# bentherien/point-cloud-reid

Hardware: AMD Instinct MI355X
Metric: siamese pair-comparisons/sec @1024 pts (higher is better)
Workload: dtype bf16x3

## Files before the change

point-cloud-reid_amd/csrc/attn_kernels_impl.h:

```cpp
#pragma once
#ifndef PCR_ATTN_PREC
#define PCR_ATTN_PREC 0
#endif
#include "tile_dense.h"

#include <stdio.h>

#include <vector>

namespace {
constexpr int kAPrec = PCR_ATTN_PREC;
struct AttnArgs {
  pcr_attn_params p;
  int dbg;
};

constexpr int kATraceWgs = 512, kATraceRecs = 24, kATraceMarks = 8;
__device__ unsigned long long g_attn_trace[2 * kATraceWgs * kATraceRecs * kATraceMarks];


__device__ __forceinline__ void pos_hidden(float *dst, int RP, const float *P, const float *w0,
                                           const float *b0, int d, int T) {
  for (int e = threadIdx.x; e < d * T; e += blockDim.x) {
    const int o = e / T, t = e - o * T;
// ... 1051 lines not shown
      bf_split8(xv, bh[s2], bl[s2], true);
    }
    PCR_AMARK(1);
    f32x16 q[ND];
#pragma unroll
    for (int cb = 0; cb < ND; cb++)
#pragma unroll
      for (int r = 0; r < 16; r++) q[cb][r] = 0.f;
    {
      const bf16x8 *wb = s_wq + lane;
#pragma unroll
      for (int s2 = 0; s2 < SQ; s2++) {
        bf16x8 wh[ND], wl[ND];
#pragma unroll
        for (int cb = 0; cb < ND; cb++) {
          wh[cb] = wb[((s2 * ND + cb) * 2) * 64];
          wl[cb] = wb[((s2 * ND + cb) * 2 + 1) * 64];
        }
#pragma unroll
        for (int cb = 0; cb < ND; cb++) q[cb] = __builtin_amdgcn_mfma_f32_32x32x16_bf16(wh[cb], bh[s2], q[cb], 0, 0, 0);
#pragma unroll
        for (int cb = 0; cb < ND; cb++) q[cb] = __builtin_amdgcn_mfma_f32_32x32x16_bf16(wh[cb], bl[s2], q[cb], 0, 0, 0);
#pragma unroll
        for (int cb = 0; cb < ND; cb++) q[cb] = __builtin_amdgcn_mfma_f32_32x32x16_bf16(wl[cb], bh[s2], q[cb], 0, 0, 0);
      }
    }
    PCR_AMARK(2);
    bf16x8 mh[SD][ND], ml[SD][ND];
    {
      const bf16x8 *mb = reinterpret_cast<const bf16x8 *>(kvp) + lane;
#pragma unroll
      for (int s2 = 0; s2 < SD; s2++)
#pragma unroll
        for (int cb = 0; cb < ND; cb++) {
          mh[s2][cb] = mb[((s2 * ND + cb) * 2) * 64];
          ml[s2][cb] = mb[((s2 * ND + cb) * 2 + 1) * 64];
        }
    }
    __builtin_amdgcn_fence(__ATOMIC_RELEASE, "wavefront");
    __builtin_amdgcn_wave_barrier();
    __builtin_amdgcn_fence(__ATOMIC_ACQUIRE, "wavefront");
    float z16[2][2] = {{0.f, 0.f}, {0.f, 0.f}};
#pragma unroll
    for (int cb = 0; cb < ND; cb++)
#pragma unroll
      for (int g = 0; g < 4; g++) {
        const f32x4 bqv = cvec(s_c, cb, g), ksv = cvec(ksw, cb, g);
        float zz = 0.f;
#pragma unroll
        for (int qq = 0; qq < 4; qq++) {
          const float v = elu1(q[cb][4 * g + qq] + bqv[qq]);
          q[cb][4 * g + qq] = v;
          zz += v * ksv[qq];
        }
        if ((g & 1) == 0) z16[cb][g >> 1] = zz;
        else z16[cb][g >> 1] += zz;
      }
    float zs[2][2];
    {
      float za = z16[0][0], zb = z16[0][1], zc = z16[1][0], zd = z16[1][1];
      if (dh >= 32) {
        za += zb; zb = za;
        zc += zd; zd = zc;
      }
      if (ND == 2 && dh >= 64) {
        za += zc; zb = za; zc = za; zd = za;
      }
      za += __shfl_xor(za, 32, 64);
      zb += __shfl_xor(zb, 32, 64);
      zc += __shfl_xor(zc, 32, 64);
      zd += __shfl_xor(zd, 32, 64);
      zs[0][0] = (1.0f / (za + 1e-6f)) * skf;
      zs[0][1] = (1.0f / (zb + 1e-6f)) * skf;
      zs[1][0] = (1.0f / (zc + 1e-6f)) * skf;
      zs[1][1] = (1.0f / (zd + 1e-6f)) * skf;
    }
#pragma unroll
    for (int cb = 0; cb < ND; cb++)
#pragma unroll
      for (int r = 0; r < 16; r++) q[cb][r] *= zs[cb][r >> 3];
    bf16x8 ch_[SD], cl_[SD];
#pragma unroll
    for (int cb = 0; cb < ND; cb++)
#pragma unroll
      for (int G = 0; G < 2; G++) to_ops(q[cb], G, ch_[2 * cb + G], cl_[2 * cb + G]);
    f32x16 m[ND];
#pragma unroll
    for (int cb = 0; cb < ND; cb++)
#pragma unroll
      for (int r = 0; r < 16; r++) m[cb][r] = 0.f;
#pragma unroll
    for (int s2 = 0; s2 < SD; s2++) {
#pragma unroll
      for (int cb = 0; cb < ND; cb++) m[cb] = __builtin_amdgcn_mfma_f32_32x32x16_bf16(mh[s2][cb], ch_[s2], m[cb], 0, 0, 0);
#pragma unroll
      for (int cb = 0; cb < ND; cb++) m[cb] = __builtin_amdgcn_mfma_f32_32x32x16_bf16(mh[s2][cb], cl_[s2], m[cb], 0, 0, 0);
#pragma unroll
      for (int cb = 0; cb < ND; cb++) m[cb] = __builtin_amdgcn_mfma_f32_32x32x16_bf16(ml[s2][cb], ch_[s2], m[cb], 0, 0, 0);
    }
    auto layernorm = [&](auto &v, auto nb_tag, const float *gam, const float *bet) __attribute__((always_inline)) {
      constexpr int NB = decltype(nb_tag)::value;
      float sm = 0.f;
#pragma unroll
      for (int cb = 0; cb < NB; cb++)
#pragma unroll
        for (int r = 0; r < 16; r++) sm += v[cb][r];
      sm += __shfl_xor(sm, 32, 64);
      const float mean = sm / (32.0f * NB);
      float vr = 0.f;
#pragma unroll
      for (int cb = 0; cb < NB; cb++)
#pragma unroll
        for (int r = 0; r < 16; r++) {
          const float dlt = v[cb][r] - mean;
          vr += dlt * dlt;
        }
      vr += __shfl_xor(vr, 32, 64);
      const float inv = 1.0f / sqrtf(vr / (32.0f * NB) + 1e-5f);
#pragma unroll
      for (int cb = 0; cb < NB; cb++)
#pragma unroll
        for (int g = 0; g < 4; g++) {
          const f32x4 gv = cvec(gam, cb, g), bv = cvec(bet, cb, g);
#pragma unroll
          for (int qq = 0; qq < 4; qq++) v[cb][4 * g + qq] = (v[cb][4 * g + qq] - mean) * inv * gv[qq] + bv[qq];
        }
    };
    PCR_AMARK(3);
    layernorm(m, std::integral_constant<int, ND>{}, s_c + 64, s_c + 128);
    PCR_AMARK(4);
#pragma unroll
    for (int s2 = 0; s2 < C1S; s2++) {
      float xv[8];
#pragma unroll
      for (int e = 0; e < 8; e++) xv[e] = xf[8 * s2 + e];
      bf_split8(xv, bh[s2], bl[s2], true);
    }
#pragma unroll
    for (int cb = 0; cb < ND; cb++)
#pragma unroll
      for (int G = 0; G < 2; G++) to_ops(m[cb], G, bh[C1S + 2 * cb + G], bl[C1S + 2 * cb + G]);
    f32x16 f[SD];
#pragma unroll
    for (int cb = 0; cb < SD; cb++)
#pragma unroll
      for (int r = 0; r < 16; r++) f[cb][r] = 0.f;
    {
      const bf16x8 *wb = s_w0 + lane;
#pragma unroll
      for (int s2 = 0; s2 < S0; s2++) {
        bf16x8 wh[SD], wl[SD];
#pragma unroll
        for (int cb = 0; cb < SD; cb++) {
          wh[cb] = wb[((s2 * SD + cb) * 2) * 64];
          wl[cb] = wb[((s2 * SD + cb) * 2 + 1) * 64];
        }
#pragma unroll
        for (int cb = 0; cb < SD; cb++) f[cb] = __builtin_amdgcn_mfma_f32_32x32x16_bf16(wh[cb], bh[s2], f[cb], 0, 0, 0);
#pragma unroll
        for (int cb = 0; cb < SD; cb++) f[cb] = __builtin_amdgcn_mfma_f32_32x32x16_bf16(wh[cb], bl[s2], f[cb], 0, 0, 0);
#pragma unroll
        for (int cb = 0; cb < SD; cb++) f[cb] = __builtin_amdgcn_mfma_f32_32x32x16_bf16(wl[cb], bh[s2], f[cb], 0, 0, 0);
      }
    }
#pragma unroll
    for (int cb = 0; cb < SD; cb++) {
#pragma unroll
      for (int r = 0; r < 16; r++) f[cb][r] = relu_i(f[cb][r]);
#pragma unroll
      for (int G = 0; G < 2; G++) to_ops(f[cb], G, bh[2 * cb + G], bl[2 * cb + G]);
    }
    PCR_AMARK(5);
    f32x16 o[NOB];
#pragma unroll
    for (int cb = 0; cb < NOB; cb++)
#pragma unroll
      for (int r = 0; r < 16; r++) o[cb][r] = 0.f;
    {
      const bf16x8 *wb = s_w2 + lane;
#pragma unroll
      for (int s2 = 0; s2 < 4 * ND; s2++) {
        bf16x8 wh[NOB], wl[NOB];
#pragma unroll
        for (int cb = 0; cb < NOB; cb++) {
          wh[cb] = wb[((s2 * NOB + cb) * 2) * 64];
          wl[cb] = wb[((s2 * NOB + cb) * 2 + 1) * 64];
        }
#pragma unroll
        for (int cb = 0; cb < NOB; cb++) o[cb] = __builtin_amdgcn_mfma_f32_32x32x16_bf16(wh[cb], bh[s2], o[cb], 0, 0, 0);
#pragma unroll
        for (int cb = 0; cb < NOB; cb++) o[cb] = __builtin_amdgcn_mfma_f32_32x32x16_bf16(wh[cb], bl[s2], o[cb], 0, 0, 0);
#pragma unroll
        for (int cb = 0; cb < NOB; cb++) o[cb] = __builtin_amdgcn_mfma_f32_32x32x16_bf16(wl[cb], bh[s2], o[cb], 0, 0, 0);
      }
    }
    PCR_AMARK(6);
    layernorm(o, std::integral_constant<int, NOB>{}, s_c + 192, s_c + 192 + 32 * NOB);
    if constexpr (C1S == 2 * NOB) {
      if (p.residual) {
#pragma unroll
        for (int cb = 0; cb < NOB; cb++)
#pragma unroll
          for (int r = 0; r < 16; r++) o[cb][r] += xf[16 * cb + r];
      }
    }
    if constexpr (POOL) {
      float vm[16], vs[16];
      {
        const bool up = (j & 1) != 0;
#pragma unroll
        for (int r = 0; r < 16; r++) {
          const float lo_ = o[r >> 4][r & 15], hi_ = o[(r + 16) >> 4][(r + 16) & 15];
          const float tk = up ? hi_ : lo_, uk = up ? lo_ : hi_;
          const float pu = __uint_as_float(pcr_sort_partner<2, 1>(__float_as_uint(uk), lane));
          vm[r] = fmaxf(tk, pu);
          vs[r] = tk + pu;
        }
      }
#define PCR_POOL_STEP(N, J, BIT)                                                                      \
      {                                                                                               \
        const bool up = (j & BIT) != 0;                                                               \
        _Pragma("unroll") for (int r = 0; r < N; r++) {                                               \
          const float tm = up ? vm[r + N] : vm[r], um = up ? vm[r] : vm[r + N];                       \
          const float ts = up ? vs[r + N] : vs[r], us = up ? vs[r] : vs[r + N];                       \
          vm[r] = fmaxf(tm, __uint_as_float(pcr_sort_partner<2 * J, J>(__float_as_uint(um), lane)));  \
          vs[r] = ts + __uint_as_float(pcr_sort_partner<2 * J, J>(__float_as_uint(us), lane));        \
        }                                                                                             \
      }
      PCR_POOL_STEP(8, 2, 2)
      PCR_POOL_STEP(4, 4, 4)
      PCR_POOL_STEP(2, 8, 8)
      PCR_POOL_STEP(1, 16, 16)
#undef PCR_POOL_STEP
      pmax = fmaxf(pmax, vm[0]);
      psum += vs[0];
      if (++pblk == nblk) {
        const int e = ((j & 1) << 4) | ((j & 2) << 2) | (j & 4) | ((j & 8) >> 2) | ((j & 16) >> 4);
        const int ch = 16 * (e >> 3) + bf_kpos(h, e & 7);
        float *po = p.pool_out + (size_t)b * 128;
        po[ch] = pmax;
        po[64 + ch] = psum;
        pmax = -INFINITY;
        psum = 0.f;
        pblk = 0;
        pc += nwav;
      }
    } else if constexpr (!CF) {
      const __amdgpu_buffer_rsrc_t rout =
          __builtin_amdgcn_make_buffer_rsrc(p.out + (size_t)b * (32 * NOB) * p.Lq, 0, 32 * NOB * p.Lq * 4, 0x00020000);
#pragma unroll
      for (int e = 0; e < 16 * NOB; e++) {
        const int ch = 16 * (e >> 3) + bf_kpos(0, e & 7);
        const float v = o[e >> 4][e & 15];
        __builtin_amdgcn_raw_buffer_store_b32(__builtin_bit_cast(unsigned, v), rout, vo, ch * p.Lq * 4, 0);
      }
    } else {
#pragma unroll
      for (int cb = 0; cb < NOB; cb++)
#pragma unroll
        for (int G = 0; G < 2; G++) to_ops(o[cb], G, bh[2 * cb + G], bl[2 * cb + G]);
      f32x16 fo[CF ? CF : 1];
#pragma unroll
      for (int cb = 0; cb < CF; cb++)
#pragma unroll
        for (int r = 0; r < 16; r++) fo[cb][r] = 0.f;
      const bf16x8 *wb = reinterpret_cast<const bf16x8 *>(p.wfinal) + lane;
#pragma unroll
      for (int s2 = 0; s2 < 2 * NOB; s2++) {
        bf16x8 wh[CF ? CF : 1], wl[CF ? CF : 1];
#pragma unroll
        for (int cb = 0; cb < CF; cb++) {
          wh[cb] = wb[((s2 * CF + cb) * 2) * 64];
          wl[cb] = wb[((s2 * CF + cb) * 2 + 1) * 64];
        }
#pragma unroll
        for (int cb = 0; cb < CF; cb++) fo[cb] = __builtin_amdgcn_mfma_f32_32x32x16_bf16(wh[cb], bh[s2], fo[cb], 0, 0, 0);
#pragma unroll
        for (int cb = 0; cb < CF; cb++) fo[cb] = __builtin_amdgcn_mfma_f32_32x32x16_bf16(wh[cb], bl[s2], fo[cb], 0, 0, 0);
#pragma unroll
        for (int cb = 0; cb < CF; cb++) fo[cb] = __builtin_amdgcn_mfma_f32_32x32x16_bf16(wl[cb], bh[s2], fo[cb], 0, 0, 0);
      }
      const __amdgpu_buffer_rsrc_t rout =
          __builtin_amdgcn_make_buffer_rsrc(p.out + (size_t)b * (32 * CF) * p.Lq, 0, 32 * CF * p.Lq * 4, 0x00020000);
#pragma unroll
      for (int cb = 0; cb < CF; cb++)
#pragma unroll
        for (int g = 0; g < 4; g++) {
          const f32x4 bv = cvec(s_c + 320, cb, g);
#pragma unroll
          for (int qq = 0; qq < 4; qq++) {
            const int e = 16 * cb + 4 * g + qq;
            const int ch = 16 * (e >> 3) + bf_kpos(0, e & 7);
            const float v = fo[cb][4 * g + qq] + bv[qq];
            __builtin_amdgcn_raw_buffer_store_b32(__builtin_bit_cast(unsigned, v), rout, vo, ch * p.Lq * 4, 0);
          }
        }
    }
    __builtin_amdgcn_wave_barrier();
    PCR_AMARK(7);
    PCR_ANEXT();
  }
#undef PCR_AMARK
#undef PCR_ANEXT
}
#endif

}

static int attn_check(const pcr_attn_params &p) {
  if (p.B < 0 || p.Lq < 1 || p.Sk < 1 || p.c1 < 1 || p.c2 < 1 || p.cout < 1 || p.nhead < 1) return 1;
  if (p.d < 32 || p.d > 512 || (p.d & 31) || p.d % p.nhead) return 1;
  if (p.d > 128 && ((p.d & 63) || ((p.d / p.nhead) & 63) || p.d / p.nhead > 256)) return 1;
  if ((p.c2 & 7) || p.cout > 512 || p.cfinal > 512) return 1;
  if (!p.feat_q || !p.feat_k || !p.xyz_k || !p.kv || !p.pos0_w || !p.pos0_b || !p.wq || !p.bq || !p.wkv ||
      !p.bkv || !p.wmerge || !p.wmlp0 || !p.wmlp2 || !p.ln1_g || !p.ln1_b || !p.ln2_g || !p.ln2_b)
    return 1;
  if (p.q_pos && (!p.xyz_q || p.c1 != p.c2 || p.c1 != p.d)) return 1;
  if (p.residual && p.cout != p.c1) return 1;
  if (p.cfinal && (!p.wfinal || !p.bfinal || (p.cout & 7))) return 1;
  return 0;
}

static void attn_dump_trace(const char *path, const char *tag, int wgs, int B, int Sk) {
  static int launches = 0;
  static const int skip = pcr_tune_int("PCR_SA_TRACE_SKIP");
  launches++;
  if (launches <= skip || launches > skip + 8) return;
  static std::vector<unsigned long long> host(2 * kATraceWgs * kATraceRecs * kATraceMarks);
  if (hipDeviceSynchronize() != hipSuccess) return;
  if (hipMemcpyFromSymbol(host.data(), HIP_SYMBOL(g_attn_trace), host.size() * sizeof(unsigned long long)) != hipSuccess) return;
  FILE *f = fopen(path, "a");
  if (!f) return;
  const int n = 2 * (wgs < kATraceWgs ? wgs : kATraceWgs);
  fprintf(f, "launch %d kernel %s wgs %d B %d Sk %d\n", launches, tag, wgs, B, Sk);
  for (int w = 0; w < n; w++) {
    const unsigned long long *t = host.data() + (size_t)w * (kATraceRecs * kATraceMarks);
    fprintf(f, "wg %d", w);
    for (int i = 0; i < kATraceRecs * kATraceMarks; i++) fprintf(f, " %llu", t[i]);
    fprintf(f, "\n");
  }
  fclose(f);
}

static int attn_kv_narrow(const pcr_attn_params *pp, pcr_stream_t stream) {
  AttnArgs a;
  a.p = *pp;
  a.dbg = 0;
  const int d = pp->d;
  if (pp->c2 < pp->d) return PCR_ERR_INVALID;
  const int tb = d <= 64 ? 2 : 1, RP = 32 * tb + 1;
  size_t lds = (size_t)(pp->c2 + d + 3) * RP + 4 * d;
  const size_t lds2 = (size_t)d * (d + 1) + d;
  if (lds2 > lds) lds = lds2;
  lds = (lds + kThreads) * sizeof(float);
  if (lds > (size_t)kMaxDynLds) return PCR_ERR_INVALID;
  static bool ok = allow_big_lds(attn_kv_kernel<2, 1, 2, 1>) && allow_big_lds(attn_kv_kernel_o3<2, 1, 1, 1>) &&
                   allow_big_lds(attn_kv_kernel_o3<1, 2, 1, 4>) && allow_big_lds(attn_kv_kernel<1, 2, 0, 4>);
  (void)ok;
  const int ntile = (pp->Sk + 32 * tb - 1) / (32 * tb);
  int ns = pp->kv_splits > 1 ? pp->kv_splits : 1;
  if (ns > 1 && (!pp->kv_part || ns > 64)) return PCR_ERR_INVALID;
  if (ns > ntile) ns = ntile;
  a.p.kv_splits = ns;
  dim3 g(pp->B, ns), blk(kThreads);
  hipStream_t st = pcr_s(stream);
  constexpr bool kBfUnit = kAPrec != 0;
  const bool bfk = kBfUnit && pp->wkv_bf != nullptr;
  if (ns == 1 && d == 64 && (pp->c2 == 64 || (pp->c2 == 128 && bfk && pp->Sk >= 128)) && (pp->Sk & 31) == 0 && pp->nhead >= 1 &&
      64 % pp->nhead == 0) {
    const bool bf = bfk;
    const bool wide = pp->c2 == 128;
    pcr_note_arith(bf ? PCR_PREC_BF16X3 : PCR_PREC_F32);
    static bool oks = allow_big_lds(attn_kv_stream64_kernel<true, false>) && allow_big_lds(attn_kv_stream64_kernel<false, false>) &&
                      allow_big_lds(attn_kv_stream64_kernel<true, kBfUnit>) && allow_big_lds(attn_kv_stream64_kernel<false, kBfUnit>) &&
                      allow_big_lds(attn_kv_stream64_kernel<true, kBfUnit, kBfUnit ? 8 : 4>) &&
                      allow_big_lds(attn_kv_stream64_kernel<false, kBfUnit, kBfUnit ? 8 : 4>);
    (void)oks;
    const int nblk = pp->Sk >> 5;
    const int minw = wide ? 4 : 2;
    int wpc2 = 1;
    while (wpc2 * 2 <= (nblk < 4 ? nblk : 4)) wpc2 *= 2;
    if (wpc2 < minw) wpc2 = minw;
    static const int no_onew = pcr_tune_int("PCR_ATTN_NO_ONEW");
    const bool onew = kBfUnit && bf && !wide && nblk <= 4 && !no_onew;
    if (onew) wpc2 = 1;
    const int cpg = kKvsWaves / wpc2;
    const size_t wu = bf ? (size_t)((wide ? 8 : 4) + 4) * 512 : 4096;
    const size_t lds_s = (wu * 4 + 256 + 128 + 64 * 65 + (onew ? (size_t)0 : (size_t)cpg * (64 * 65 + 64))) * sizeof(float);
    const long rounds = ((long)pp->B + cpg - 1) / cpg;
    static const int ncu = [] {
      hipDeviceProp_t pr;
      int dev = 0;
      if (hipGetDevice(&dev) != hipSuccess || hipGetDeviceProperties(&pr, dev) != hipSuccess) return 256;
      return pr.multiProcessorCount > 0 ? pr.multiProcessorCount : 256;
    }();
    const int gs = (int)(rounds < ncu ? rounds : ncu);
    const dim3 gg(gs), bb(64 * kKvsWaves);
    if (bf && wide) {
      if (pp->nhead >= 2) hipLaunchKernelGGL((attn_kv_stream64_kernel<true, kBfUnit, kBfUnit ? 8 : 4>), gg, bb, lds_s, st, a);
      else hipLaunchKernelGGL((attn_kv_stream64_kernel<false, kBfUnit, kBfUnit ? 8 : 4>), gg, bb, lds_s, st, a);
    } else if (bf) {
      static const char *atrace = pcr_tune_str("PCR_ATTN_TRACE");
      if (atrace) a.dbg |= 256;
      if (onew) {
        static bool oko = allow_big_lds(attn_kv_stream64_kernel<true, kBfUnit, 4, kBfUnit>) &&
                          allow_big_lds(attn_kv_stream64_kernel<false, kBfUnit, 4, kBfUnit>);
        (void)oko;
        if (pp->nhead >= 2) hipLaunchKernelGGL((attn_kv_stream64_kernel<true, kBfUnit, 4, kBfUnit>), gg, bb, lds_s, st, a);
        else hipLaunchKernelGGL((attn_kv_stream64_kernel<false, kBfUnit, 4, kBfUnit>), gg, bb, lds_s, st, a);
      } else if (pp->nhead >= 2) hipLaunchKernelGGL((attn_kv_stream64_kernel<true, kBfUnit>), gg, bb, lds_s, st, a);
      else hipLaunchKernelGGL((attn_kv_stream64_kernel<false, kBfUnit>), gg, bb, lds_s, st, a);
      if (atrace) attn_dump_trace(atrace, "kv64", gs, (int)pp->B, pp->Sk);
    } else {
      if (pp->nhead >= 2) hipLaunchKernelGGL((attn_kv_stream64_kernel<true, false>), gg, bb, lds_s, st, a);
      else hipLaunchKernelGGL((attn_kv_stream64_kernel<false, false>), gg, bb, lds_s, st, a);
    }
    PCR_CHECK_LAUNCH();
    return PCR_OK;
  }
#if PCR_ATTN_PREC != 0
  if (ns == 1 && d == 32 && pp->c2 == 32 && pp->wkv_bf && (pp->Sk & 31) == 0 && pp->nhead >= 1 && 32 % pp->nhead == 0) {
    static bool ok32 = allow_big_lds(attn_kv_stream32_kernel);
    (void)ok32;
    pcr_note_arith(PCR_PREC_BF16X3);
    const int nblk = pp->Sk >> 5;
    int wpc2 = 1;
    while (wpc2 * 2 <= (nblk < kKvsWaves ? nblk : kKvsWaves)) wpc2 *= 2;
    if (wpc2 < 2) wpc2 = 2;
    const int cpg = kKvsWaves / wpc2;
    const size_t lds_s = (size_t)(4096 + 128 + 64 + 32 * 33 + cpg * (32 * 33 + 32)) * sizeof(float);
    const long rounds = ((long)pp->B + cpg - 1) / cpg;
    static const int ncu = [] {
      hipDeviceProp_t pr;
      int dev = 0;
      if (hipGetDevice(&dev) != hipSuccess || hipGetDeviceProperties(&pr, dev) != hipSuccess) return 256;
      return pr.multiProcessorCount > 0 ? pr.multiProcessorCount : 256;
    }();
    const long cap = 2L * ncu;
    hipLaunchKernelGGL(attn_kv_stream32_kernel, dim3((unsigned)(rounds < cap ? rounds : cap)), dim3(64 * kKvsWaves), lds_s, st, a);
    PCR_CHECK_LAUNCH();
    return PCR_OK;
  }
#endif
  pcr_note_arith(PCR_PREC_F32);
  if (d == 32) hipLaunchKernelGGL((attn_kv_kernel<2, 1, 2, 1>), g, blk, lds, st, a);
  else if (d == 64) hipLaunchKernelGGL((attn_kv_kernel_o3<2, 1, 1, 1>), g, blk, lds, st, a);
  else if (d == 128) {
    static bool ok2 = allow_big_lds(attn_kv_kernel_o2<1, 2, 1, 4>) && allow_big_lds(attn_kv_kernel_o2<1, 2, 1, 4, true>);
    (void)ok2;
    if (kBfUnit && pp->wkv_bf && pp->Sk >= 256) hipLaunchKernelGGL((attn_kv_kernel_o2<1, 2, 1, 4, true>), g, blk, lds, st, a);
    else hipLaunchKernelGGL((attn_kv_kernel_o2<1, 2, 1, 4>), g, blk, lds, st, a);
  }
  else hipLaunchKernelGGL((attn_kv_kernel<1, 2, 0, 4>), g, blk, lds, st, a);
  PCR_CHECK_LAUNCH();
  if (ns > 1) {
    static bool okf = allow_big_lds(attn_kv_fold_kernel);
    (void)okf;
    hipLaunchKernelGGL(attn_kv_fold_kernel, dim3(pp->B), blk, ((size_t)d * (d + 1) + d) * sizeof(float), st, a);
    PCR_CHECK_LAUNCH();
  }
  return PCR_OK;
}

static int attn_apply_launch(const pcr_attn_params *pp, pcr_stream_t stream) {
  const pcr_attn_params &p = *pp;
  AttnArgs a;
  a.p = p;
  a.dbg = 0;
  const int tb = p.d <= 32 ? 4 : (p.d <= 64 ? 2 : 1), T = 32 * tb, RP = T + 1;
  const int catP = ceil8(p.c1 + p.d);
  int rowsU = catP > 2 * p.d ? catP : 2 * p.d;
  if (ceil32(p.cout) > rowsU) rowsU = ceil32(p.cout);
  if (ceil32(p.cfinal) > rowsU) rowsU = ceil32(p.cfinal);
  size_t lds = ((size_t)(rowsU + 3 + p.nhead) * RP + 2 * (kThreads / T) * T + 7 * p.d + 2 * p.cout) *
               sizeof(float);
  if (lds > (size_t)kMaxDynLds) return PCR_ERR_INVALID;
  dim3 g((p.Lq + T - 1) / T, p.B), blk(kThreads);
  hipStream_t st = pcr_s(stream);
  pcr_note_arith(kAPrec != 0 ? PCR_PREC_BF16X3 : PCR_PREC_F32);
#if PCR_ATTN_PREC != 0
  const int aps_c1s = (p.c1 + 15) >> 4, aps_nd = p.d >> 5;
  const size_t aps_lds = (size_t)((aps_c1s + (p.q_pos ? 2 * aps_nd : 0)) * aps_nd * 128 + (aps_c1s + 2 * aps_nd) * aps_nd * 256 +
                                  aps_nd * (p.cout >> 5) * 512) * 16 +
                         (size_t)(448 + 256 + 64 * kApsWaves) * sizeof(float);
  if (p.d == 32 && p.c1 == 32 && p.cout == 32 && !p.cfinal && (p.Lq & 31) == 0 && (p.nhead == 1 || p.nhead == 2)) {
    const long nitem = (long)p.B * (p.Lq >> 5);
    const long nwg = (nitem + kApsWaves - 1) / kApsWaves;
    static const int ncu = [] {
      hipDeviceProp_t pr;
      int dev = 0;
      if (hipGetDevice(&dev) != hipSuccess || hipGetDeviceProperties(&pr, dev) != hipSuccess) return 256;
      return pr.multiProcessorCount > 0 ? pr.multiProcessorCount : 256;
    }();
    const dim3 gg((unsigned)(nwg < ncu ? nwg : ncu)), bb(64 * kApsWaves);
    static bool ok32 = allow_big_lds(attn_apply_stream64_kernel<true, 2, 0, 1, 1>) && allow_big_lds(attn_apply_stream64_kernel<false, 2, 0, 1, 1>);
    (void)ok32;
    if (p.q_pos) hipLaunchKernelGGL((attn_apply_stream64_kernel<true, 2, 0, 1, 1>), gg, bb, aps_lds, st, a);
    else hipLaunchKernelGGL((attn_apply_stream64_kernel<false, 2, 0, 1, 1>), gg, bb, aps_lds, st, a);
    PCR_CHECK_LAUNCH();
    return PCR_OK;
  }
  const bool aps_in = p.c1 == 64 || ((p.c1 == 32 || (p.c1 < 16 && pp->wmlp0_bf_xpad)) && !p.q_pos && !p.residual);
  const bool aps_out = (p.cout == 64 && (p.cfinal == 0 || p.cfinal == 128) && p.c1 >= 32) ||
                       (p.cout == 128 && !p.cfinal && !p.residual && p.c1 == 64) ||
                       (p.cout == 32 && p.cfinal == 64 && !p.residual && p.c1 < 16);
  if (p.d == 64 && aps_in && aps_out &&
      (p.Lq & 31) == 0 && (p.nhead == 1 || p.nhead == 2 || p.nhead == 4) && aps_lds <= (size_t)kMaxDynLds) {
    const int c1s = aps_c1s, sq = c1s + (p.q_pos ? 4 : 0), s0 = c1s + 4;
    const int nob = p.cout >> 5;
    const size_t lds_s = (size_t)(sq * 256 + s0 * 512 + nob * 1024) * 16 + (size_t)(448 + 256 + 64 * kApsWaves) * sizeof(float);
    const long nitem = (long)p.B * (p.Lq >> 5);
    const long nwg = (nitem + kApsWaves - 1) / kApsWaves;
    static const int ncu = [] {
      hipDeviceProp_t pr;
      int dev = 0;
      if (hipGetDevice(&dev) != hipSuccess || hipGetDeviceProperties(&pr, dev) != hipSuccess) return 256;
      return pr.multiProcessorCount > 0 ? pr.multiProcessorCount : 256;
    }();
    const dim3 gg((unsigned)(nwg < ncu ? nwg : ncu)), bb(64 * kApsWaves);
#define PCR_APS(QP, C1Sv, CFv)                                                            \
  do {                                                                                    \
    static bool oks = allow_big_lds(attn_apply_stream64_kernel<QP, C1Sv, CFv>);           \
    (void)oks;                                                                            \
    hipLaunchKernelGGL((attn_apply_stream64_kernel<QP, C1Sv, CFv>), gg, bb, lds_s, st, a); \
  } while (0)
    const bool cf = p.cfinal != 0;
    static const char *aptrace = pcr_tune_str("PCR_ATTN_TRACE");
    if (aptrace) a.dbg = 256;
    if (pp->pool_out) {
      static bool okp = allow_big_lds(attn_apply_stream64_kernel<false, 4, 0, 2, 2, true>);
      (void)okp;
      const long nwgp = ((long)p.B + kApsWaves - 1) / kApsWaves;
      const dim3 ggp((unsigned)(nwgp < ncu ? nwgp : ncu));
      hipLaunchKernelGGL((attn_apply_stream64_kernel<false, 4, 0, 2, 2, true>), ggp, bb, lds_s, st, a);
      PCR_CHECK_LAUNCH();
      return PCR_OK;
    }
    if (nob == 4) {
      static bool ok4 = allow_big_lds(attn_apply_stream64_kernel<true, 4, 0, 4>) && allow_big_lds(attn_apply_stream64_kernel<false, 4, 0, 4>);
      (void)ok4;
      if (p.q_pos) hipLaunchKernelGGL((attn_apply_stream64_kernel<true, 4, 0, 4>), gg, bb, lds_s, st, a);
      else hipLaunchKernelGGL((attn_apply_stream64_kernel<false, 4, 0, 4>), gg, bb, lds_s, st, a);
    } else if (p.c1 < 16) {
      static bool ok1 = allow_big_lds(attn_apply_stream64_kernel<false, 1, 2, 1>);
      (void)ok1;
      hipLaunchKernelGGL((attn_apply_stream64_kernel<false, 1, 2, 1>), gg, bb, lds_s, st, a);
    } else if (p.c1 == 32) { if (cf) PCR_APS(false, 2, 4); else PCR_APS(false, 2, 0); }
    else if (p.q_pos) { if (cf) PCR_APS(true, 4, 4); else PCR_APS(true, 4, 0); }
    else { if (cf) PCR_APS(false, 4, 4); else PCR_APS(false, 4, 0); }
#undef PCR_APS
    if (aptrace) attn_dump_trace(aptrace, "apply64", (int)gg.x, (int)p.B, p.Lq);
    PCR_CHECK_LAUNCH();
    return PCR_OK;
  }
#endif
  const bool wide = 2 * p.d > 128 || p.cout > 128 || p.cfinal > 128;
#define PCR_APPLY(TBv, NRv)                                                          \
  do {                                                                               \
    static bool ok = allow_big_lds(attn_apply_kernel<TBv, NRv>);                     \
    (void)ok;                                                                        \
    hipLaunchKernelGGL((attn_apply_kernel<TBv, NRv>), g, blk, lds, st, a);           \
  } while (0)
  if (tb == 4) {
    if (wide) PCR_APPLY(4, 2);
    else PCR_APPLY(4, 1);
  } else if (tb == 2) {
    if (wide) PCR_APPLY(2, 2);
    else PCR_APPLY(2, 1);
  } else {
    int widest = 2 * p.d > p.cout ? 2 * p.d : p.cout;
    if (p.cfinal > widest) widest = p.cfinal;
#if PCR_ATTN_PREC == 0
    if (widest > 512) PCR_APPLY(1, 8);
    else if (widest > 256) PCR_APPLY(1, 4);
    else PCR_APPLY(1, 2);
#else
    if (widest > 256) return PCR_ERR_INVALID;
    PCR_APPLY(1, 2);
#endif
  }
#undef PCR_APPLY
  PCR_CHECK_LAUNCH();
  return PCR_OK;
}

#if PCR_ATTN_PREC == 1
int pcr_attn_kv_bf3(const pcr_attn_params *pp, pcr_stream_t stream) { return attn_kv_narrow(pp, stream); }
int pcr_attn_apply_bf3(const pcr_attn_params *pp, pcr_stream_t stream) { return attn_apply_launch(pp, stream); }
#else
int pcr_attn_kv_bf3(const pcr_attn_params *pp, pcr_stream_t stream);
int pcr_attn_apply_bf3(const pcr_attn_params *pp, pcr_stream_t stream);

static bool attn_bf(const pcr_attn_params &p, pcr_attn_params &q) {
  const int widest = 2 * p.d > p.cout ? (2 * p.d > p.cfinal ? 2 * p.d : p.cfinal) : (p.cout > p.cfinal ? p.cout : p.cfinal);
  if (p.precision == 0 || p.d > 128 || widest > 256 || !p.wq_bf || !p.wmlp0_bf || !p.wmlp2_bf ||
      (p.cfinal && !p.wfinal_bf))
    return false;
  q = p;
  q.wq = p.wq_bf; q.wmlp0 = p.wmlp0_bf; q.wmlp2 = p.wmlp2_bf; q.wfinal = p.wfinal_bf;
  return true;
}

PCR_EXPORT int pcr_attn_kv_splits(int B, int Sk, int d) {
  (void)B;
  if (Sk < 1 || d > 64) return 1;
  if ((d == 64 || d == 32) && (Sk & 31) == 0) return 1;
  const int ntile = (Sk + 63) / 64;
  return ntile >= 16 ? 4 : (ntile >= 8 ? 2 : 1);
}

PCR_EXPORT int pcr_attn_kv_f32(const pcr_attn_params *pp, pcr_stream_t stream) {
  if (!pp || attn_check(*pp)) return PCR_ERR_INVALID;
  if (pp->B == 0) return PCR_OK;
  const int d = pp->d;
  if (d > 128) {
    AttnArgs a;
    a.p = *pp;
    a.dbg = 0;
    if (!pp->wkv_wide || !pp->bkv_wide || !pp->wmerge_packed || pp->B > 65535) return PCR_ERR_INVALID;
    pcr_note_arith(PCR_PREC_F32);
    const int dh = d / pp->nhead;
    size_t lds = ((size_t)(pp->c2 + d + 3) * 33 + 4 * d + kThreads) * sizeof(float);
    const size_t lds2 = (size_t)dh * 65 * sizeof(float);
    if (lds2 > lds) lds = lds2;
    if (lds > (size_t)kMaxDynLds) return PCR_ERR_INVALID;
    static bool okw = allow_big_lds(attn_kv_wide_kernel<2>) && allow_big_lds(attn_kv_wide_kernel<3>);
    (void)okw;
    dim3 g(d / 64, pp->B), blk(kThreads);
    if (64 + dh <= 256) hipLaunchKernelGGL((attn_kv_wide_kernel<2>), g, blk, lds, pcr_s(stream), a);
    else hipLaunchKernelGGL((attn_kv_wide_kernel<3>), g, blk, lds, pcr_s(stream), a);
    PCR_CHECK_LAUNCH();
    return PCR_OK;
  }
  pcr_attn_params q;
  if (attn_bf(*pp, q)) return pcr_attn_kv_bf3(&q, stream);
  return attn_kv_narrow(pp, stream);
}

static bool attn_pool_ok(const pcr_attn_params &p) {
  pcr_attn_params q;
  return p.d == 64 && p.c1 == 64 && p.cout == 64 && !p.cfinal && !p.q_pos && (p.Lq & 31) == 0 &&
         (p.nhead == 1 || p.nhead == 2 || p.nhead == 4) && attn_bf(p, q);
}

PCR_EXPORT int pcr_attn_apply_pool_ok(const pcr_attn_params *pp) {
  return (pp && !attn_check(*pp) && attn_pool_ok(*pp)) ? 1 : 0;
}

PCR_EXPORT int pcr_attn_apply_f32(const pcr_attn_params *pp, pcr_stream_t stream) {
  if (!pp || attn_check(*pp) || (!pp->out && !pp->pool_out)) return PCR_ERR_INVALID;
  if (pp->pool_out && !attn_pool_ok(*pp)) return PCR_ERR_INVALID;
  if (pp->B == 0) return PCR_OK;
  if (pp->B > 65535) return PCR_ERR_INVALID;
  pcr_attn_params q;
  if (attn_bf(*pp, q)) return pcr_attn_apply_bf3(&q, stream);
  return attn_apply_launch(pp, stream);
}
#endif
```

Before: 64410.

## Add persistent streaming attention-apply kernel for d=128 with LDS weight ring

Adds a persistent kernel specialised for d=128 attention apply, where each wave processes one 32-point block end to end. It covers the Q projection, linear-attention KV product, both layernorms, the MLP and the residual, all with bf16x3 MFMA. Weights are streamed through a double-buffered LDS ring in chunks shared by the waves of a workgroup, and the grid is capped at the CU count. The goal is to replace the generic tiled path and its intermediate traffic for this shape, at the cost of one wave per EU, high register pressure, and a syncthreads per chunk.

After: 65990 (median of 6 runs). +2.5%, better.

```diff
diff --git a/point-cloud-reid_amd/csrc/attn_kernels_impl.h b/point-cloud-reid_amd/csrc/attn_kernels_impl.h
--- a/point-cloud-reid_amd/csrc/attn_kernels_impl.h
+++ b/point-cloud-reid_amd/csrc/attn_kernels_impl.h
@@ -1377,6 +1377,302 @@
   }
 #undef PCR_AMARK
 #undef PCR_ANEXT
+}
+
+template <int NB>
+__device__ __forceinline__ void ap128_step(f32x16 (&acc)[NB], const bf16x8 *wb, int ls, const bf16x8 &bh, const bf16x8 &bl) {
+#pragma unroll
+  for (int c0 = 0; c0 < NB; c0 += 4) {
+    bf16x8 wh[4], wl[4];
+#pragma unroll
+    for (int cb = 0; cb < 4; cb++) {
+      wh[cb] = wb[((ls * NB + c0 + cb) * 2) * 64];
+      wl[cb] = wb[((ls * NB + c0 + cb) * 2 + 1) * 64];
+    }
+#pragma unroll
+    for (int cb = 0; cb < 4; cb++) acc[c0 + cb] = __builtin_amdgcn_mfma_f32_32x32x16_bf16(wh[cb], bh, acc[c0 + cb], 0, 0, 0);
+#pragma unroll
+    for (int cb = 0; cb < 4; cb++) acc[c0 + cb] = __builtin_amdgcn_mfma_f32_32x32x16_bf16(wh[cb], bl, acc[c0 + cb], 0, 0, 0);
+#pragma unroll
+    for (int cb = 0; cb < 4; cb++) acc[c0 + cb] = __builtin_amdgcn_mfma_f32_32x32x16_bf16(wl[cb], bh, acc[c0 + cb], 0, 0, 0);
+    asm volatile("" ::: "memory");
+  }
+}
+constexpr int kAp128Waves = 4, kAp128ChunkU = 2048, kAp128Chunks = 16;
+constexpr size_t kAp128Lds = (size_t)2 * kAp128ChunkU * 16 + (640 + 4 * 128 + kAp128Waves * 128) * sizeof(float);
+template <int NH>
+__global__ __launch_bounds__(64 * kAp128Waves) __attribute__((amdgpu_waves_per_eu(1, 1)))
+void attn_apply_stream128_kernel(AttnArgs a) {
+  constexpr int D = 128, ND = 4, SD = 8, GPH = 8 / NH;
+  constexpr int NPC = kAp128ChunkU / (64 * kAp128Waves);
+  extern __shared__ __attribute__((aligned(16))) float smem[];
+  const pcr_attn_params &p = a.p;
+  f32x4 *s_ring = reinterpret_cast<f32x4 *>(smem);
+  int coff = 2 * kAp128ChunkU * 4;
+  asm volatile("" : "+s"(coff));
+  float *s_c = smem + coff;
+  f32x4 *s_p0 = reinterpret_cast<f32x4 *>(s_c + 640);
+  float *s_ks = s_c + 640 + 4 * 128;
+  const int tid = threadIdx.x, lane = tid & 63, j = lane & 31, h = lane >> 5;
+  const int wave = __builtin_amdgcn_readfirstlane(tid >> 6);
+  const __amdgpu_buffer_rsrc_t rwq = __builtin_amdgcn_make_buffer_rsrc(const_cast<float *>(p.wq), 0, 4 * kAp128ChunkU * 16, 0x00020000),
+                               rw0 = __builtin_amdgcn_make_buffer_rsrc(const_cast<float *>(p.wmlp0), 0, 8 * kAp128ChunkU * 16, 0x00020000),
+                               rw2 = __builtin_amdgcn_make_buffer_rsrc(const_cast<float *>(p.wmlp2), 0, 4 * kAp128ChunkU * 16, 0x00020000);
+  f32x4 stg[NPC];
+  auto fetch = [&](int k) __attribute__((always_inline)) {
+    k %= kAp128Chunks;
+    const __amdgpu_buffer_rsrc_t r = k < 4 ? rwq : (k < 12 ? rw0 : rw2);
+    const int kk = k < 4 ? k : (k < 12 ? k - 4 : k - 12);
+#pragma unroll
+    for (int u = 0; u < NPC; u++)
+      stg[u] = __builtin_bit_cast(f32x4, __builtin_amdgcn_raw_buffer_load_b128(r, tid * 16, (kk * kAp128ChunkU + u * 64 * kAp128Waves) * 16, 0));
+    asm volatile("" ::: "memory");
+  };
+  auto commit = [&](int k) __attribute__((always_inline)) {
+    f32x4 *dst = s_ring + (k & 1) * kAp128ChunkU + tid;
+#pragma unroll
+    for (int u = 0; u < NPC; u++) dst[u * 64 * kAp128Waves] = stg[u];
+    __syncthreads();
+  };
+  for (int e = tid; e < D; e += 64 * kAp128Waves) {
+    s_c[e] = p.bq[e];
+    s_c[128 + e] = p.ln1_g[e];
+    s_c[256 + e] = p.ln1_b[e];
+    s_c[384 + e] = p.ln2_g[e];
+    s_c[512 + e] = p.ln2_b[e];
+    s_p0[e] = f32x4{p.pos0_w[3 * e], p.pos0_w[3 * e + 1], p.pos0_w[3 * e + 2], p.pos0_b[e]};
+  }
+  fetch(0);
+  commit(0);
+  const int nblk = p.Lq >> 5;
+  const long nitem = (long)p.B * nblk;
+  const float skf = (float)p.Sk;
+  float *ksw = s_ks + wave * 128;
+  auto cvec = [&](const float *base, int cb, int g) __attribute__((always_inline)) {
+    return *reinterpret_cast<const f32x4 *>(base + 32 * cb + 8 * g + 4 * h);
+  };
+  auto to_ops = [&](const f32x16 &acc, int G, bf16x8 &oh, bf16x8 &ol) __attribute__((always_inline)) {
+    float v[8];
+#pragma unroll
+    for (int e = 0; e < 8; e++) v[e] = acc[8 * G + e];
+    bf_split8(v, oh, ol, true);
+  };
+  auto layernorm = [&](f32x16 (&v)[ND], const float *gam, const float *bet) __attribute__((always_inline)) {
+    float sm = 0.f;
+#pragma unroll
+    for (int cb = 0; cb < ND; cb++)
+#pragma unroll
+      for (int r = 0; r < 16; r++) sm += v[cb][r];
+    sm += __shfl_xor(sm, 32, 64);
+    const float mean = sm / (float)D;
+    float vr = 0.f;
+#pragma unroll
+    for (int cb = 0; cb < ND; cb++)
+#pragma unroll
+      for (int r = 0; r < 16; r++) {
+        const float dlt = v[cb][r] - mean;
+        vr += dlt * dlt;
+      }
+    vr += __shfl_xor(vr, 32, 64);
+    const float inv = 1.0f / sqrtf(vr / (float)D + 1e-5f);
+#pragma unroll
+    for (int cb = 0; cb < ND; cb++)
+#pragma unroll
+      for (int g = 0; g < 4; g++) {
+        const f32x4 gv = cvec(gam, cb, g), bv = cvec(bet, cb, g);
+#pragma unroll
+        for (int qq = 0; qq < 4; qq++) v[cb][4 * g + qq] = (v[cb][4 * g + qq] - mean) * inv * gv[qq] + bv[qq];
+      }
+  };
+  for (long it0 = (long)blockIdx.x * kAp128Waves; it0 < nitem; it0 += (long)gridDim.x * kAp128Waves) {
+    const long item = it0 + wave;
+    const bool live = item < nitem;
+    const long it = live ? item : nitem - 1;
+    const long b = it / nblk;
+    const int blk = (int)(it - b * nblk);
+    const size_t bq_ = p.q_index ? (size_t)p.q_index[b] : (size_t)b;
+    const size_t kb_ = p.kv_index ? (size_t)p.kv_index[b] : (size_t)b;
+    const float *kvp = p.kv + kb_ * ((size_t)D * D + D);
+    const int t = blk * 32 + j;
+    const __amdgpu_buffer_rsrc_t rfeat = __builtin_amdgcn_make_buffer_rsrc(
+        const_cast<float *>(p.feat_q + bq_ * D * p.Lq), 0, D * p.Lq * 4, 0x00020000);
+    const int vo = (4 * h * p.Lq + t) * 4;
+    auto load_x = [&](float (&xf)[64]) __attribute__((always_inline)) {
+#pragma unroll
+      for (int e = 0; e < 64; e++) {
+        const int ch = 16 * (e >> 3) + bf_kpos(0, e & 7);
+        xf[e] = __builtin_bit_cast(float, __builtin_amdgcn_raw_buffer_load_b32(rfeat, vo, ch * p.Lq * 4, 0));
+      }
+    };
+    ksw[lane] = kvp[(size_t)D * D + lane];
+    ksw[64 + lane] = kvp[(size_t)D * D + 64 + lane];
+    bf16x8 bh[16], bl[16];
+    {
+      float xf[64];
+      load_x(xf);
+      const float *xyz = p.xyz_q + (bq_ * p.Lq + t) * 3;
+      const float px = xyz[0], py = xyz[1], pz = xyz[2];
+#pragma unroll
+      for (int s2 = 0; s2 < SD; s2++) {
+        float hv[8];
+#pragma unroll
+        for (int e = 0; e < 8; e++) {
+          const f32x4 w = s_p0[16 * s2 + bf_kpos(0, e) + 4 * h];
+          const float v = w[0] * px + w[1] * py + w[2] * pz + w[3];
+          hv[e] = relu_i(v);
+        }
+        bf_split8(hv, bh[SD + s2], bl[SD + s2], true);
+      }
+#pragma unroll
+      for (int e = 0; e < 64; e++) asm volatile("" : "+v"(xf[e]));
+#pragma unroll
+      for (int s2 = 0; s2 < SD; s2++) {
+        float xv[8];
+#pragma unroll
+        for (int e = 0; e < 8; e++) xv[e] = xf[8 * s2 + e];
+        bf_split8(xv, bh[s2], bl[s2], true);
+      }
+    }
+    f32x16 q[ND];
+#pragma unroll
+    for (int cb = 0; cb < ND; cb++)
+#pragma unroll
+      for (int g = 0; g < 4; g++) {
+        const f32x4 bqv = cvec(s_c, cb, g);
+#pragma unroll
+        for (int qq = 0; qq < 4; qq++) q[cb][4 * g + qq] = bqv[qq];
+      }
+#pragma unroll
+    for (int k = 0; k < 4; k++) {
+      fetch(k + 1);
+      const bf16x8 *wb = reinterpret_cast<const bf16x8 *>(s_ring + (k & 1) * kAp128ChunkU) + lane;
+#pragma unroll
+      for (int ls = 0; ls < 4; ls++) ap128_step<ND>(q, wb, ls, bh[4 * k + ls], bl[4 * k + ls]);
+      commit(k + 1);
+    }
+    float zg[SD];
+#pragma unroll
+    for (int cb = 0; cb < ND; cb++)
+#pragma unroll
+      for (int g = 0; g < 4; g++) {
+        const f32x4 ksv = cvec(ksw, cb, g);
+        float zz = 0.f;
+#pragma unroll
+        for (int qq = 0; qq < 4; qq++) {
+          const float v = elu1(q[cb][4 * g + qq]);
+          q[cb][4 * g + qq] = v;
+          zz += v * ksv[qq];
+        }
+        if ((g & 1) == 0) zg[2 * cb + (g >> 1)] = zz;
+        else zg[2 * cb + (g >> 1)] += zz;
+      }
+    float zs[NH];
+#pragma unroll
+    for (int hd = 0; hd < NH; hd++) {
+      float z = zg[hd * GPH];
+#pragma unroll
+      for (int gi = 1; gi < GPH; gi++) z += zg[hd * GPH + gi];
+      z += __shfl_xor(z, 32, 64);
+      zs[hd] = (1.0f / (z + 1e-6f)) * skf;
+    }
+#pragma unroll
+    for (int cb = 0; cb < ND; cb++)
+#pragma unroll
+      for (int r = 0; r < 16; r++) q[cb][r] *= zs[(2 * cb + (r >> 3)) / GPH];
+    {
+      bf16x8 ch_[SD], cl_[SD];
+#pragma unroll
+      for (int cb = 0; cb < ND; cb++)
+#pragma unroll
+        for (int G = 0; G < 2; G++) to_ops(q[cb], G, ch_[2 * cb + G], cl_[2 * cb + G]);
+#pragma unroll
+      for (int cb = 0; cb < ND; cb++)
+#pragma unroll
+        for (int r = 0; r < 16; r++) q[cb][r] = 0.f;
+      const bf16x8 *mb = reinterpret_cast<const bf16x8 *>(kvp) + lane;
+      bf16x8 mh[2][ND], ml[2][ND];
+#pragma unroll
+      for (int cb = 0; cb < ND; cb++) {
+        mh[0][cb] = mb[(cb * 2) * 64];
+        ml[0][cb] = mb[(cb * 2 + 1) * 64];
+      }
+#pragma unroll
+      for (int s2 = 0; s2 < SD; s2++) {
+        const int c = s2 & 1;
+        if (s2 + 1 < SD) {
+#pragma unroll
+          for (int cb = 0; cb < ND; cb++) {
+            mh[c ^ 1][cb] = mb[(((s2 + 1) * ND + cb) * 2) * 64];
+            ml[c ^ 1][cb] = mb[(((s2 + 1) * ND + cb) * 2 + 1) * 64];
+          }
+        }
+        asm volatile("" ::: "memory");
+#pragma unroll
+        for (int cb = 0; cb < ND; cb++) q[cb] = __builtin_amdgcn_mfma_f32_32x32x16_bf16(mh[c][cb], ch_[s2], q[cb], 0, 0, 0);
+#pragma unroll
+        for (int cb = 0; cb < ND; cb++) q[cb] = __builtin_amdgcn_mfma_f32_32x32x16_bf16(mh[c][cb], cl_[s2], q[cb], 0, 0, 0);
+#pragma unroll
+        for (int cb = 0; cb < ND; cb++) q[cb] = __builtin_amdgcn_mfma_f32_32x32x16_bf16(ml[c][cb], ch_[s2], q[cb], 0, 0, 0);
+      }
+    }
+    layernorm(q, s_c + 128, s_c + 256);
+#pragma unroll
+    for (int cb = 0; cb < ND; cb++)
+#pragma unroll
+      for (int G = 0; G < 2; G++) to_ops(q[cb], G, bh[SD + 2 * cb + G], bl[SD + 2 * cb + G]);
+    f32x16 f[2 * ND];
+#pragma unroll
+    for (int cb = 0; cb < 2 * ND; cb++)
+#pragma unroll
+      for (int r = 0; r < 16; r++) f[cb][r] = 0.f;
+#pragma unroll
+    for (int k = 4; k < 12; k++) {
+      fetch(k + 1);
+      const bf16x8 *wb = reinterpret_cast<const bf16x8 *>(s_ring + (k & 1) * kAp128ChunkU) + lane;
+#pragma unroll
+      for (int ls = 0; ls < 2; ls++) ap128_step<2 * ND>(f, wb, ls, bh[2 * (k - 4) + ls], bl[2 * (k - 4) + ls]);
+      commit(k + 1);
+    }
+    float xf[64];
+    load_x(xf);
+    f32x16 o[ND];
+#pragma unroll
+    for (int cb = 0; cb < ND; cb++)
+#pragma unroll
+      for (int r = 0; r < 16; r++) o[cb][r] = 0.f;
+#pragma unroll
+    for (int k = 12; k < 16; k++) {
+      fetch(k + 1);
+      bf16x8 oh[4], ol[4];
+#pragma unroll
+      for (int i = 0; i < 2; i++) {
+        f32x16 &fc = f[2 * (k - 12) + i];
+#pragma unroll
+        for (int r = 0; r < 16; r++) fc[r] = relu_i(fc[r]);
+#pragma unroll
+        for (int G = 0; G < 2; G++) to_ops(fc, G, oh[2 * i + G], ol[2 * i + G]);
+      }
+      const bf16x8 *wb = reinterpret_cast<const bf16x8 *>(s_ring + (k & 1) * kAp128ChunkU) + lane;
+#pragma unroll
+      for (int ls = 0; ls < 4; ls++) ap128_step<ND>(o, wb, ls, oh[ls], ol[ls]);
+      commit(k + 1);
+    }
+    layernorm(o, s_c + 384, s_c + 512);
+#pragma unroll
+    for (int cb = 0; cb < ND; cb++)
+#pragma unroll
+      for (int r = 0; r < 16; r++) o[cb][r] += xf[16 * cb + r];
+    if (live) {
+      const __amdgpu_buffer_rsrc_t rout =
+          __builtin_amdgcn_make_buffer_rsrc(p.out + (size_t)b * D * p.Lq, 0, D * p.Lq * 4, 0x00020000);
+#pragma unroll
+      for (int e = 0; e < 16 * ND; e++) {
+        const int ch = 16 * (e >> 3) + bf_kpos(0, e & 7);
+        const float v = o[e >> 4][e & 15];
+        __builtin_amdgcn_raw_buffer_store_b32(__builtin_bit_cast(unsigned, v), rout, vo, ch * p.Lq * 4, 0);
+      }
+    }
+  }
 }
 #endif
 
@@ -1558,6 +1854,27 @@
   const size_t aps_lds = (size_t)((aps_c1s + (p.q_pos ? 2 * aps_nd : 0)) * aps_nd * 128 + (aps_c1s + 2 * aps_nd) * aps_nd * 256 +
                                   aps_nd * (p.cout >> 5) * 512) * 16 +
                          (size_t)(448 + 256 + 64 * kApsWaves) * sizeof(float);
+  static const int no_s128 = pcr_tune_int("PCR_ATTN_NO_STREAM128");
+  if (p.d == 128 && p.c1 == 128 && p.cout == 128 && !p.cfinal && p.q_pos && p.residual && (p.Lq & 31) == 0 && p.Lq >= 256 &&
+      (p.nhead == 1 || p.nhead == 2 || p.nhead == 4) && !no_s128) {
+    const long nitem = (long)p.B * (p.Lq >> 5);
+    const long nwg = (nitem + kAp128Waves - 1) / kAp128Waves;
+    static const int ncu = [] {
+      hipDeviceProp_t pr;
+      int dev = 0;
+      if (hipGetDevice(&dev) != hipSuccess || hipGetDeviceProperties(&pr, dev) != hipSuccess) return 256;
+      return pr.multiProcessorCount > 0 ? pr.multiProcessorCount : 256;
+    }();
+    const dim3 gg((unsigned)(nwg < ncu ? nwg : ncu)), bb(64 * kAp128Waves);
+    static bool ok128 = allow_big_lds(attn_apply_stream128_kernel<1>) && allow_big_lds(attn_apply_stream128_kernel<2>) &&
+                        allow_big_lds(attn_apply_stream128_kernel<4>);
+    (void)ok128;
+    if (p.nhead == 1) hipLaunchKernelGGL((attn_apply_stream128_kernel<1>), gg, bb, kAp128Lds, st, a);
+    else if (p.nhead == 2) hipLaunchKernelGGL((attn_apply_stream128_kernel<2>), gg, bb, kAp128Lds, st, a);
+    else hipLaunchKernelGGL((attn_apply_stream128_kernel<4>), gg, bb, kAp128Lds, st, a);
+    PCR_CHECK_LAUNCH();
+    return PCR_OK;
+  }
   if (p.d == 32 && p.c1 == 32 && p.cout == 32 && !p.cfinal && (p.Lq & 31) == 0 && (p.nhead == 1 || p.nhead == 2)) {
     const long nitem = (long)p.B * (p.Lq >> 5);
     const long nwg = (nitem + kApsWaves - 1) / kApsWaves;
```
